# louiskirsch/speechT

Hardware: AMD Instinct MI355X
Metric: utterances/sec (training step, 10 s@16 kHz, batch 32) (higher is better)
Workload: dtype f32

## Files before the change

### include/speecht_hip.h

```cpp
#ifndef SPEECHT_HIP_H
#define SPEECHT_HIP_H

#include <stddef.h>
#include <stdint.h>

#ifdef __cplusplus
extern "C" {
#endif

#define ST_OK 0
#define ST_EINVAL (-1)
#define ST_ELAUNCH (-2)
#define ST_EWORKSPACE (-3)
#define ST_ECOMM (-4)

typedef struct st_tensor3 {
  float* base;
  int32_t batch;
  int32_t frames;
  int32_t channels;
  int32_t halo;
  int32_t t_pitch;
  int32_t c_pitch;
} st_tensor3;
// ... 10 lines not shown

int st_packed_dims(int width, int cin_pitch, int cout, int* k_valid, int* k_pad, int* n_pad);
int st_pack_filters_f32(const float* filters, int width, int cin, int cout, int cin_pitch,
                        float* packed, void* stream);
int st_unpack_filters_f32(const float* packed, int width, int cin, int cout, int cin_pitch,
                          float* filters, void* stream);
int st_filters_flip_transpose_f32(const float* packed, int width, int cin, int cout,
                                  int cin_pitch, int cout_pitch, float* packed_t, void* stream);

int st_conv1d_nwc_fwd_f32(const st_tensor3* x, const float* packed, const float* bias, int width,
                          int stride, int pad_left, int relu, const st_tensor3* y, void* stream);
size_t st_conv1d_fwd_ws(const st_tensor3* x, const st_tensor3* y, int width);
int st_conv1d_nwc_fwd_ws_f32(const st_tensor3* x, const float* packed, const float* bias, int width,
                             int stride, int pad_left, int relu, const st_tensor3* y, void* workspace,
                             size_t workspace_bytes, void* stream);

int st_conv1d_fft_plan(int width, int frames, int batch, int* n, int* valid, int* blocks, int* bins, int* rows_pad);
int st_gemm_nn_batched_f32(const float* a, int64_t lda, int64_t a_batch, const float* b, int64_t b_batch, float* c,
                           int64_t ldc, int64_t c_batch, int m, int k, int n, int batches, void* stream);
size_t st_gemm_nn_batched_ws_bytes(void);
size_t st_gemm_nn_batched_ctrl_bytes(void);
int st_streamk_lost_ptr(void** device_word);
int st_streamk_lost_count(unsigned* count);
int st_streamk_lost_fetch_async(unsigned* host_word, void* stream);
int st_gemm_nn_batched_ws_f32(const float* a, int64_t lda, int64_t a_batch, const float* b, int64_t b_batch, float* c,
                              int64_t ldc, int64_t c_batch, int m, int k, int n, int batches, void* workspace,
                              size_t workspace_bytes, void* stream);
int st_gemm_nn_batched_bt_ws_f32(const float* a, int64_t lda, int64_t a_batch, const float* bt, int64_t bt_batch, float* c,
                                 int64_t ldc, int64_t c_batch, int m, int k, int n, int batches, void* workspace,
                                 size_t workspace_bytes, void* stream);
// ... 51 lines not shown
                                      const float* tables, int planes, void* workspace, size_t workspace_bytes, void* stream);
int st_conv1d_nwc_bwd_filter_fft_planes(const st_tensor3* x, const st_tensor3* dz, const void* sf_planes, const void* zf_planes, int width,
                                        const float* tables, float* dpacked, int planes, void* workspace, size_t workspace_bytes,
                                        void* stream);

size_t st_conv1d_bwd_data_ws(const st_tensor3* dz, const st_tensor3* dx, int width);
int st_conv1d_nwc_bwd_data_f32(const st_tensor3* dz, const float* packed_t, int width,
                               int pad_left, const st_tensor3* act, const st_tensor3* dx,
                               void* workspace, size_t workspace_bytes, void* stream);
size_t st_conv1d_bwd_data_bias_ws(const st_tensor3* dz, const st_tensor3* dx, int width);
int st_conv1d_nwc_bwd_data_bias_f32(const st_tensor3* dz, const float* packed_t, int width, int pad_left,
                                    const st_tensor3* act, const st_tensor3* dx, float* dbias_dx,
                                    void* workspace, size_t workspace_bytes, void* stream);
int st_conv1d_1tap_bwd_data_bias_f32(const st_tensor3* dz, const float* packed, const st_tensor3* act, const st_tensor3* dx,
                                     float* dbias_dx, void* workspace, size_t workspace_bytes, void* stream);
size_t st_conv1d_bwd_filter_ws(const st_tensor3* x, const st_tensor3* dz, int width);
size_t st_bias_grad_ws(const st_tensor3* dz);
int st_bias_grad_f32(const st_tensor3* dz, float* dbias, void* workspace, size_t workspace_bytes, void* stream);
int st_conv1d_nwc_bwd_filter_f32(const st_tensor3* x, const st_tensor3* dz, int width, int stride,
                                 int pad_left, float* dpacked, float* dbias, void* workspace,
                                 size_t workspace_bytes, void* stream);

size_t st_ctc_ws(int batch, int frames, int max_label_len);
int st_ctc_loss_grad_f32(const st_tensor3* logits, const int32_t* label_ids,
                         const int32_t* label_offsets, const int32_t* seq_lens, int max_label_len,
                         float grad_scale, float* loss, const st_tensor3* grad, int32_t* status,
                         void* workspace, size_t workspace_bytes, void* stream);
int st_ctc_loss_grad_hilo_f32(const st_tensor3* logits, const int32_t* label_ids,
                              const int32_t* label_offsets, const int32_t* seq_lens, int max_label_len,
                              float grad_scale, float* loss, float* loss_lo, const st_tensor3* grad, int32_t* status,
// ... 144 lines not shown
```

### speecht_amd/_lib.py

```python
import ctypes
import os
from ctypes import POINTER, c_char_p, c_float, c_int, c_int32, c_int64, c_size_t, c_void_p

from .build import LIB_PATH


class Tensor3(ctypes.Structure):
  _fields_ = [('base', c_void_p), ('batch', c_int32), ('frames', c_int32), ('channels', c_int32),
              ('halo', c_int32), ('t_pitch', c_int32), ('c_pitch', c_int32)]


class SpeechtHipError(RuntimeError):
  pass


_T3P = POINTER(Tensor3)
_SIGNATURES = {
    'st_version': (c_int, []),
    'st_last_error': (c_char_p, []),
    'st_trace_begin': (c_int, []),
    'st_trace_begin_timed': (c_int, []),
    'st_trace_timed_filter': (c_int, [c_char_p]),
    'st_trace_end': (c_size_t, [c_char_p, c_size_t]),
    'st_set_tuning': (c_int, [c_char_p, c_int]),
    'st_host_crc32c': (ctypes.c_uint32, [c_void_p, c_size_t, ctypes.c_uint32]),
    'st_packed_dims': (c_int, [c_int, c_int, c_int, POINTER(c_int), POINTER(c_int), POINTER(c_int)]),
    'st_pack_filters_f32': (c_int, [c_void_p, c_int, c_int, c_int, c_int, c_void_p, c_void_p]),
    'st_unpack_filters_f32': (c_int, [c_void_p, c_int, c_int, c_int, c_int, c_void_p, c_void_p]),
    'st_filters_flip_transpose_f32': (c_int, [c_void_p, c_int, c_int, c_int, c_int, c_int, c_void_p, c_void_p]),
    'st_conv1d_nwc_fwd_f32': (c_int, [_T3P, c_void_p, c_void_p, c_int, c_int, c_int, c_int, _T3P, c_void_p]),
    'st_conv1d_fwd_ws': (c_size_t, [_T3P, _T3P, c_int]),
    'st_conv1d_nwc_fwd_ws_f32': (c_int, [_T3P, c_void_p, c_void_p, c_int, c_int, c_int, c_int, _T3P, c_void_p, c_size_t,
                                          c_void_p]),
    'st_conv1d_fft_plan': (c_int, [c_int, c_int, c_int, POINTER(c_int), POINTER(c_int), POINTER(c_int), POINTER(c_int),
                                   POINTER(c_int)]),
    'st_gemm_nn_batched_f32': (c_int, [c_void_p, c_int64, c_int64, c_void_p, c_int64, c_void_p, c_int64, c_int64, c_int, c_int,
                                       c_int, c_int, c_void_p]),
    'st_gemm_nn_batched_ws_bytes': (c_size_t, []),
    'st_gemm_nn_batched_ctrl_bytes': (c_size_t, []),
    'st_streamk_lost_ptr': (c_int, [POINTER(c_void_p)]),
    'st_streamk_lost_count': (c_int, [POINTER(ctypes.c_uint32)]),
    'st_streamk_lost_fetch_async': (c_int, [c_void_p, c_void_p]),
    'st_gemm_nn_batched_ws_f32': (c_int, [c_void_p, c_int64, c_int64, c_void_p, c_int64, c_void_p, c_int64, c_int64, c_int, c_int,
                                          c_int, c_int, c_void_p, c_size_t, c_void_p]),
    'st_gemm_nn_batched_bt_ws_f32': (c_int, [c_void_p, c_int64, c_int64, c_void_p, c_int64, c_void_p, c_int64, c_int64, c_int, c_int,
                                             c_int, c_int, c_void_p, c_size_t, c_void_p]),
    'st_gemm_tn_batched_f32': (c_int, [c_void_p, c_int64, c_int64, c_void_p, c_int64, c_int64, c_void_p, c_int64, c_int, c_int,
                                       c_int, c_int, c_void_p]),
# ... 28 lines not shown
                                                  c_void_p, c_size_t, c_void_p]),
    'st_conv1d_nwc_bwd_filter_fft_planes': (c_int, [_T3P, _T3P, c_void_p, c_void_p, c_int, c_void_p, c_void_p, c_int, c_void_p, c_size_t,
                                                    c_void_p]),
    'st_conv1d_fft_dz_spectra_f32': (c_int, [_T3P, c_int, c_void_p, c_void_p, c_void_p]),
    'st_conv1d_fft_bias_grad_f32': (c_int, [_T3P, c_int, c_void_p, c_void_p, c_void_p]),
    'st_conv1d_nwc_bwd_data_fft_f32': (c_int, [_T3P, c_void_p, c_void_p, c_int, c_int, _T3P, _T3P, c_void_p, c_void_p, c_size_t,
                                               c_void_p]),
    'st_conv1d_nwc_bwd_filter_fft_f32': (c_int, [_T3P, _T3P, c_void_p, c_void_p, c_int, c_void_p, c_void_p, c_void_p,
                                                 c_size_t, c_void_p]),
    'st_conv1d_bwd_data_ws': (c_size_t, [_T3P, _T3P, c_int]),
    'st_conv1d_nwc_bwd_data_f32': (c_int, [_T3P, c_void_p, c_int, c_int, _T3P, _T3P, c_void_p, c_size_t, c_void_p]),
    'st_conv1d_bwd_data_bias_ws': (c_size_t, [_T3P, _T3P, c_int]),
    'st_conv1d_nwc_bwd_data_bias_f32': (c_int, [_T3P, c_void_p, c_int, c_int, _T3P, _T3P, c_void_p, c_void_p, c_size_t,
                                                c_void_p]),
    'st_conv1d_1tap_bwd_data_bias_f32': (c_int, [_T3P, c_void_p, _T3P, _T3P, c_void_p, c_void_p, c_size_t, c_void_p]),
    'st_conv1d_bwd_filter_ws': (c_size_t, [_T3P, _T3P, c_int]),
    'st_conv1d_nwc_bwd_filter_f32': (c_int, [_T3P, _T3P, c_int, c_int, c_int, c_void_p, c_void_p, c_void_p,
                                             c_size_t, c_void_p]),
    'st_bias_grad_ws': (c_size_t, [_T3P]),
    'st_bias_grad_f32': (c_int, [_T3P, c_void_p, c_void_p, c_size_t, c_void_p]),
    'st_ctc_ws': (c_size_t, [c_int, c_int, c_int]),
    'st_ctc_loss_grad_f32': (c_int, [_T3P, c_void_p, c_void_p, c_void_p, c_int, c_float, c_void_p, _T3P,
                                     c_void_p, c_void_p, c_size_t, c_void_p]),
    'st_ctc_loss_grad_hilo_f32': (c_int, [_T3P, c_void_p, c_void_p, c_void_p, c_int, c_float, c_void_p, c_void_p, _T3P,
                                     c_void_p, c_void_p, c_size_t, c_void_p]),
    'st_ctc_greedy_decode': (c_int, [_T3P, c_void_p, c_int, c_void_p, c_int, c_void_p, c_void_p, c_void_p]),
    'st_ctc_align_ws': (c_size_t, [c_int, c_int, c_int]),
    'st_ctc_align_f32': (c_int, [_T3P, c_void_p, c_void_p, c_void_p, c_int, c_void_p, c_void_p, c_void_p, c_void_p,
                                 c_void_p, c_size_t, c_void_p]),
    'st_ctc_align_host': (c_int, [c_void_p, c_int, c_int, c_int, c_void_p, c_void_p, c_void_p, c_int, c_void_p, c_void_p,
# ... 159 lines not shown
```

### speecht_amd/csrc/conv_gemm.hip

```cpp
#include <algorithm>
#include <atomic>
#include <cmath>
#include <cstdlib>

#include <type_traits>

#include "st_common.h"
#include "streamk_map.h"

namespace {

typedef float f32x16 __attribute__((ext_vector_type(16)));
typedef float f32x4 __attribute__((ext_vector_type(4)));

constexpr int BK = 32;
constexpr int APITCH = BK + 4;
constexpr int NTHREADS = 256;

struct RowMap {
  int frames;
  int row_stride;
  long batch_stride;
  long row0;
  __device__ __forceinline__ long off(int m) const {
// ... 8 lines not shown
  const float* Bm; int Np;
  float* C;        RowMap cmap;
  const float* mask; RowMap mmap;
  const float* bias;
  int M, Kvalid, Kp, n_store, relu;
  int taps, cp;
  int tiles_m, tiles_n, chunk;
  int gm, tm_per, tn_per;
  int splits, steps_per_split;
  float* slab;
  float* colsum;
  int colsum_rows;
  int batches;
  long a_batch, b_batch, c_batch;
  long bt_ld; int bt_rows;
};


__device__ __forceinline__ void dma16_sv(unsigned lds_byte_addr, const void* sbase, unsigned voff_bytes) {
  unsigned keep;
  asm volatile("s_mov_b32 %0, m0\n\ts_mov_b32 m0, %1\n\ts_nop 0\n\tglobal_load_lds_dwordx4 %2, %3\n\ts_mov_b32 m0, %0"
               : "=&s"(keep) : "s"(lds_byte_addr), "v"(voff_bytes), "s"(sbase) : "memory");
}
__device__ __forceinline__ void dma_wait_all() { asm volatile("s_waitcnt vmcnt(0)" ::: "memory"); }
__device__ __forceinline__ unsigned lds_addr(const float* p) {
  return (unsigned)(size_t)(__attribute__((address_space(3))) const float*)p;
}

template <int N> struct FVec;
template <> struct FVec<1> { typedef float type; };
// ... 89 lines not shown
  for (; kt + 2 < nk; kt += 2) {
    stage(integral_constant<int, 0>{}, true_type{});
    stage(integral_constant<int, 1>{}, true_type{});
  }
  if (kt + 2 == nk) {
    stage(integral_constant<int, 0>{}, true_type{});
    stage(integral_constant<int, 1>{}, false_type{});
  } else if (kt + 1 == nk) {
    stage(integral_constant<int, 0>{}, false_type{});
  }
}

template <int BM, int BN, int WMW, int WNW, int EPI, bool FAST = false, bool BT = false>
__global__ __launch_bounds__(NTHREADS) void gemm_nn_kernel(NNParams p) {
  static_assert(!BT || FAST, "the transposed-operand variant exists for whole k-tiles only");
  typedef NNStage<BM, BN, WMW, WNW, BT> S;
  constexpr int WTM = S::WTM, WTN = S::WTN, MT = S::MT, NT = S::NT;
  constexpr int A_DMA = S::A_DMA, B_DMA = S::B_DMA, N_DMA = S::N_DMA, A_SZ = S::A_SZ, B_SZ = S::B_SZ;
  constexpr int B_LPR = BN / 4;
  static_assert(WMW * WNW == 4 && MT >= 1 && (NT == 1 || NT == 2 || NT == 4) && A_DMA >= 1 && B_DMA >= 1, "tile config");
  typedef typename FVec<NT>::type bvec;

  __shared__ __attribute__((aligned(16))) float smem[2 * A_SZ + 2 * B_SZ + 6 * BM];
  float* const As = smem;
  float* const Bs = smem + 2 * A_SZ;
  long* const a_off = reinterpret_cast<long*>(smem + 2 * A_SZ + 2 * B_SZ);
  long* const c_off = a_off + BM;
  long* const m_off = c_off + BM;

  const int bid = blockIdx.x;
// ... 130 lines not shown
        for (int r = 0; r < 16; ++r) {
          const int m = m0 + wm * WTM + i * 32 + (r & 3) + 8 * (r >> 2) + 4 * h;
          if (m < p.M) {
#pragma unroll
            for (int n = 0; n < NT; ++n) slab[(long)m * p.Np + colb + n * 32] = acc[i][n][r];
          }
        }
      return;
    }
    float csum[NT], bv[NT];
    bool ok[NT];
#pragma unroll
    for (int n = 0; n < NT; ++n) {
      ok[n] = colb + n * 32 < p.n_store;
      csum[n] = 0.f;
      bv[n] = (EPI == 0 && p.bias && ok[n]) ? p.bias[colb + n * 32] : 0.f;
    }
#pragma unroll
    for (int i = 0; i < MT; ++i) {
      float mk[16][NT];
      if (EPI == 1 && p.mask) {
#pragma unroll
        for (int r = 0; r < 16; ++r) {
          const int row = wm * WTM + i * 32 + (r & 3) + 8 * (r >> 2) + 4 * h;
#pragma unroll
          for (int n = 0; n < NT; ++n) mk[r][n] = p.mask[m_off[row] + (ok[n] ? colb + n * 32 : 0)];
        }
      }
#pragma unroll
      for (int r = 0; r < 16; ++r) {
        const int row = wm * WTM + i * 32 + (r & 3) + 8 * (r >> 2) + 4 * h;
        const long co = c_off[row];
#pragma unroll
        for (int n = 0; n < NT; ++n) {
          float v = acc[i][n][r];
          if (EPI == 0) {
            v += bv[n];
            if (p.relu) v = fmaxf(v, 0.f);
          } else if (p.mask) {
            v = mk[r][n] > 0.f ? v : 0.f;
          }
          if (co >= 0 && ok[n]) {
            if (EPI == 1) csum[n] += v;
            Cbase[co + colb + n * 32] = v;
          }
        }
      }
    }
    if (EPI == 1 && p.colsum) {
#pragma unroll
      for (int n = 0; n < NT; ++n) {
// ... 14 lines not shown
        if (m < p.M) {
          bvec out;
#pragma unroll
          for (int n = 0; n < NT; ++n) vset<NT>(out, n, acc[i][n][r]);
          *reinterpret_cast<bvec*>(slab + (long)m * p.Np + col0) = out;
        }
      }
    return;
  }
  const bool col_ok = col0 < p.n_store;
  float csum[NT];
#pragma unroll
  for (int n = 0; n < NT; ++n) csum[n] = 0.f;
  bvec bv;
#pragma unroll
  for (int n = 0; n < NT; ++n) vset<NT>(bv, n, (EPI == 0 && p.bias && col_ok) ? p.bias[col0 + n] : 0.f);
#pragma unroll
  for (int i = 0; i < MT; ++i) {
    bvec mk[16];
    if (EPI == 1 && p.mask) {
      const int colc = col_ok ? col0 : 0;
#pragma unroll
      for (int r = 0; r < 16; ++r) {
        const int row = wm * WTM + i * 32 + (r & 3) + 8 * (r >> 2) + 4 * h;
        mk[r] = *reinterpret_cast<const bvec*>(p.mask + m_off[row] + colc);
      }
    }
#pragma unroll
    for (int r = 0; r < 16; ++r) {
      const int row = wm * WTM + i * 32 + (r & 3) + 8 * (r >> 2) + 4 * h;
      const long co = c_off[row];
      if (co >= 0 && col_ok) {
        bvec out;
#pragma unroll
        for (int n = 0; n < NT; ++n) {
          float v = acc[i][n][r];
          if (EPI == 0) {
            v += vget<NT>(bv, n);
            if (p.relu) v = fmaxf(v, 0.f);
          } else if (p.mask) {
            v = vget<NT>(mk[r], n) > 0.f ? v : 0.f;
          }
          if (EPI == 1) csum[n] += v;
          vset<NT>(out, n, v);
        }
        *reinterpret_cast<bvec*>(Cbase + co + col0) = out;
      }
    }
  }
  if (EPI == 1 && p.colsum) {
    bvec out;
#pragma unroll
    for (int n = 0; n < NT; ++n) vset<NT>(out, n, csum[n] + __shfl_xor(csum[n], 32, 64));
    if (h == 0) *reinterpret_cast<bvec*>(p.colsum + (long)(tile_m * WMW + wm) * p.Np + col0) = out;
  }
}

__device__ unsigned g_sk_lost = 0;

struct BinsParams {
  const float* A; const float* B; float* C;
  long lda, ldb, ldc, a_batch, b_batch, c_batch;
// ... 785 lines not shown
    const float* src = p.slab + (long)m * p.Np + c4;
    f32x4 v = *reinterpret_cast<const f32x4*>(src);
    for (int sidx = 1; sidx < p.splits; ++sidx) v += *reinterpret_cast<const f32x4*>(src + (long)sidx * p.M * p.Np);
    if (epi == 0) {
      if (p.bias) v += *reinterpret_cast<const f32x4*>(p.bias + c4);
      if (p.relu) { v[0] = fmaxf(v[0], 0.f); v[1] = fmaxf(v[1], 0.f); v[2] = fmaxf(v[2], 0.f); v[3] = fmaxf(v[3], 0.f); }
    } else if (p.mask) {
      f32x4 mk = *reinterpret_cast<const f32x4*>(p.mask + p.mmap.off(m) + c4);
#pragma unroll
      for (int e = 0; e < 4; ++e) v[e] = mk[e] > 0.f ? v[e] : 0.f;
    }
    *reinterpret_cast<f32x4*>(p.C + p.cmap.off(m) + c4) = v;
  }
}

int nn_splits(int M, int Np, int Kp) {
  if (Np % 128) return 1;
  const long tiles128 = (long)st::ceil_div(M, 128) * (Np / 128);
  const int nk = Kp / BK;
  int splits = tiles128 < 64 && nk >= 256 ? (int)std::min<long>(8, 256 / tiles128)
                                          : (tiles128 > 128 && tiles128 <= 320 && nk >= 512 ? 2 : 1);
  while (splits > 1 && nk / splits < 64) --splits;
  return splits;
}

int fwd_splits(int M, int Np, int nk) {
  if (Np == 32) {
    if (M < 1024 || nk < 32) return 1;
    const int tiles_m = st::ceil_div(M, 128);
    return std::max(1, std::min(std::min(8, nk / 4), (512 + tiles_m / 2) / tiles_m));
// ... 25 lines not shown
    p.chunk = p.tm_per * p.tn_per;
  }
  p.colsum_rows = p.tiles_m * WMW;
  if (p.batches > 0) p.chunk = st::ceil_div(p.batches, 8) * p.tiles_m * p.tiles_n;
  dim3 grid(p.chunk * 8, p.splits > 1 ? p.splits : 1), block(NTHREADS);
  const double gflop = 2e-9 * p.tiles_m * BM * (double)p.Np * p.Kp * std::max(1, p.batches);
  if (p.batches > 0)
    st::trace("gemm_nn<%d,%d,%d,%d,%s> batched bins=%d M=%d Np=%d Kp=%d gflop=%.3f", BM, BN, WMW, WNW, FAST ? (BT ? "fast-bt" : "fast") : "clamped",
              p.batches, p.M, p.Np, p.Kp, gflop);
  else
    st::trace("gemm_nn<%d,%d,%d,%d,%s> epi=%d splits=%d M=%d Np=%d Kp=%d taps=%d xcd=%dx%d gflop=%.3f", BM, BN, WMW, WNW,
              FAST ? (BT ? "fast-bt" : "fast") : "clamped", epi, p.splits > 1 ? p.splits : 1, p.M, p.Np, p.Kp, p.taps, p.gm, 8 / p.gm, gflop);
  {
    st::LaunchTimer timer(s);
    if (epi == 0) st::launch_timed(timer, gemm_nn_kernel<BM, BN, WMW, WNW, 0, FAST, BT>, grid, block, s, p);
    else st::launch_timed(timer, gemm_nn_kernel<BM, BN, WMW, WNW, 1, FAST, BT>, grid, block, s, p);
  }
  if (p.splits > 1) {
    const long quads = (long)p.M * (p.n_store / 4);
    hipLaunchKernelGGL(splitk_epilogue_kernel, dim3((unsigned)std::min<long>((quads + 255) / 256, 4096)), dim3(256), 0, s,
                       p, epi);
  }
}

int run_nn(NNParams& p, int epi, hipStream_t s) {
  if (p.bt_ld > 0) {
    if (!(p.Np % 128 == 0 && p.taps == 1 && p.cp % 32 == 0 && p.Kvalid % 32 == 0 && p.Kvalid == p.Kp && p.bt_ld % 4 == 0 && p.bt_rows > 0)) {
      st::set_error("gemm_nn: the transposed-operand form needs n_pad %% 128 == 0, one tap and a reduction length that is a multiple of 32");
      return ST_EINVAL;
    }
    const long tiles128 = (long)st::ceil_div(p.M, 128) * (p.Np / 128) * std::max(1, p.batches);
    if ((p.batches > 0 && (tiles128 < 512 || p.M <= 64)) || (p.batches <= 0 && tiles128 < 192 && p.splits <= 1)) launch_nn<64, 128, 2, 2, true, true>(p, epi, s);
    else launch_nn<128, 128, 2, 2, true, true>(p, epi, s);
// ... 176 lines not shown
  TN3Params p{};
  p.A = A; p.lda = lda; p.a_batch = a_batch;
  p.Z = Z; p.ldz = ldz; p.z_batch = z_batch;
  for (int i = 0; i < 3; ++i) { p.a_off[i] = a_off[i]; p.z_off[i] = z_off[i]; }
  p.out = out; p.o_batch = o_batch; p.o_part = o_part;
  p.M = M; p.K = K; p.N = N; p.tiles_k = K / 128; p.tiles_n = N / 128; p.batches = batches;
  st::trace("gemm_tn_g3<128> batched bins=%d M=%d Kp=%d Np=%d gflop=%.3f", batches, M, K, N, 2e-9 * 3 * M * (double)K * N * batches);
  st::LaunchTimer timer(s);
  st::launch_timed(timer, gemm_tn_g3_kernel, dim3(st::ceil_div(batches, 8) * p.tiles_k * p.tiles_n * 8), dim3(TN_THREADS), s, p);
  return st::check_launch("gemm_tn_g3_batched");
}

static int bwd_data_impl(const st_tensor3* dz, const float* packed_t, bool forward_filters, int width, int pad_left,
                         const st_tensor3* act, const st_tensor3* dx, float* dbias_dx, void* workspace,
                         size_t workspace_bytes, void* stream);

extern "C" {

int st_streamk_lost_ptr(void** device_word) {
  ST_REQUIRE(device_word, "st_streamk_lost_ptr: null argument");
  void* p = nullptr;
  if (hipGetSymbolAddress(&p, HIP_SYMBOL(g_sk_lost)) != hipSuccess || !p) {
    st::set_error("st_streamk_lost_ptr: hipGetSymbolAddress failed");
    return ST_ELAUNCH;
  }
  *device_word = p;
  return ST_OK;
}

int st_streamk_lost_fetch_async(unsigned* host_word, void* stream) {
// ... 94 lines not shown
  const int np = st::npad_of(y->channels);
  const int M = y->batch * y->frames;
  const int nk = width > 1 ? st::ceil_div(x->c_pitch, BK) * width : st::ceil_div(x->c_pitch, BK);
  const int splits = fwd_splits(M, np, nk);
  return splits > 1 ? (size_t)splits * M * np * sizeof(float) : 0;
}

int st_conv1d_nwc_fwd_f32(const st_tensor3* x, const float* packed, const float* bias, int width,
                          int stride, int pad_left, int relu, const st_tensor3* y, void* stream) {
  return st_conv1d_nwc_fwd_ws_f32(x, packed, bias, width, stride, pad_left, relu, y, nullptr, 0, stream);
}

int st_conv1d_nwc_fwd_ws_f32(const st_tensor3* x, const float* packed, const float* bias, int width,
                             int stride, int pad_left, int relu, const st_tensor3* y, void* workspace,
                             size_t workspace_bytes, void* stream) {
  ST_REQUIRE(st::tensor_ok(x) && st::tensor_ok(y) && packed, "conv fwd: bad tensor descriptor");
  ST_REQUIRE(width > 0 && stride > 0 && pad_left >= 0 && x->batch == y->batch, "conv fwd: bad shape");
  ST_REQUIRE(y->frames == st::ceil_div(x->frames, stride), "conv fwd: y.frames != ceil(x.frames/stride)");
  ST_REQUIRE(x->halo >= pad_left, "conv fwd: x.halo %d < pad_left %d", x->halo, pad_left);
  ST_REQUIRE((y->frames - 1) * stride + width - pad_left <= x->t_pitch - x->halo,
             "conv fwd: trailing halo of x too small");
  NNParams p{};
  p.A = x->base;
  p.amap = make_map(*x, x->halo - pad_left, stride, y->frames);
  p.Bm = packed;
  p.Np = st::npad_of(y->channels);
  p.C = y->base;
  p.cmap = make_map(*y, y->halo, 1, y->frames);
  p.bias = bias;
  p.M = y->batch * y->frames;
  p.Kvalid = width * x->c_pitch;
  p.Kp = (int)st::round_up(p.Kvalid, BK);
  p.n_store = std::min(y->c_pitch, p.Np);
  p.relu = relu;
  p.taps = width;
  p.cp = x->c_pitch;
  const int nk = p.taps > 1 ? st::ceil_div(p.cp, BK) * p.taps : p.Kp / BK;
  const int splits = fwd_splits(p.M, p.Np, nk);
  if (splits > 1 && workspace && workspace_bytes >= (size_t)splits * p.M * p.Np * sizeof(float)) {
    p.steps_per_split = st::ceil_div(nk, splits);
    p.splits = st::ceil_div(nk, p.steps_per_split);
    p.slab = reinterpret_cast<float*>(workspace);
  }
  return run_nn(p, 0, st::as_stream(stream));
}

size_t st_conv1d_bwd_data_ws(const st_tensor3* dz, const st_tensor3* dx, int width) {
  if (!dz || !dx) return 0;
  const int np = st::npad_of(dx->channels), kp = (int)st::round_up((size_t)width * dz->c_pitch, BK);
  const int M = dx->batch * dx->frames;
  const int splits = nn_splits(M, np, kp);
  return splits > 1 ? (size_t)splits * M * np * sizeof(float) : 0;
}

int st_conv1d_nwc_bwd_data_f32(const st_tensor3* dz, const float* packed_t, int width, int pad_left,
                               const st_tensor3* act, const st_tensor3* dx, void* workspace,
                               size_t workspace_bytes, void* stream) {
  return st_conv1d_nwc_bwd_data_bias_f32(dz, packed_t, width, pad_left, act, dx, nullptr, workspace, workspace_bytes, stream);
}

// ... 4 lines not shown
  return st::round_up(st_conv1d_bwd_data_ws(dz, dx, width), 256) + rows * np * sizeof(float) + 256;
}

int st_conv1d_nwc_bwd_data_bias_f32(const st_tensor3* dz, const float* packed_t, int width, int pad_left,
                                    const st_tensor3* act, const st_tensor3* dx, float* dbias_dx, void* workspace,
                                    size_t workspace_bytes, void* stream) {
  return bwd_data_impl(dz, packed_t, false, width, pad_left, act, dx, dbias_dx, workspace, workspace_bytes, stream);
}

int st_conv1d_1tap_bwd_data_bias_f32(const st_tensor3* dz, const float* packed, const st_tensor3* act, const st_tensor3* dx,
                                     float* dbias_dx, void* workspace, size_t workspace_bytes, void* stream) {
  ST_REQUIRE(st::tensor_ok(dz) && st::tensor_ok(dx) && dz->c_pitch % 32 == 0 && st::npad_of(dx->channels) % 128 == 0 &&
                 st::npad_of(dz->channels) >= dz->c_pitch,
             "conv 1-tap bwd_data: needs a channel pitch of dz that is a multiple of 32 and an input width that packs to 128s");
  return bwd_data_impl(dz, packed, true, 1, 0, act, dx, dbias_dx, workspace, workspace_bytes, stream);
}

}

static int bwd_data_impl(const st_tensor3* dz, const float* packed_t, bool forward_filters, int width, int pad_left,
                         const st_tensor3* act, const st_tensor3* dx, float* dbias_dx, void* workspace,
                         size_t workspace_bytes, void* stream) {
  ST_REQUIRE(st::tensor_ok(dz) && st::tensor_ok(dx) && packed_t, "conv bwd_data: bad tensor descriptor");
  ST_REQUIRE(dz->batch == dx->batch && dz->frames == dx->frames, "conv bwd_data: stride-1 layers only");
  const int lead = width - 1 - pad_left;
  ST_REQUIRE(lead >= 0 && dz->halo >= lead, "conv bwd_data: dz.halo %d < %d", dz->halo, lead);
  ST_REQUIRE(dz->frames + pad_left <= dz->t_pitch - dz->halo, "conv bwd_data: trailing halo of dz too small");
  if (act) ST_REQUIRE(st::tensor_ok(act) && act->batch == dx->batch && act->frames == dx->frames &&
                      act->c_pitch >= std::min(dx->c_pitch, st::npad_of(dx->channels)),
                      "conv bwd_data: mask tensor mismatch");
// ... 162 lines not shown
```

### speecht_amd/modes/fp32.py

```python
import ctypes
import os
from types import SimpleNamespace

import torch

from .. import _lib
from .._lib import call
from .base import ModeBase
from .spectral import SpectralLayers


class Fp32Mode(SpectralLayers, ModeBase):
  _one_tap_in_place = True
  _flip_every_layer = False
  masks_padding = True

  def __init__(self, engine):
    super().__init__(engine)
    self._packed_t_fresh, self._packed_t_layers, self._bwd_ready = False, frozenset(), {}
    self._gfwd_fresh, self._gfwd_ready, self._fft_table_key, self._fft_prev = False, {}, {}, None

  def weights_changed(self):
    self._packed_t_fresh = False
    self._gfwd_fresh = False
# ... 3 lines not shown

  def alloc(self, sh):
    lib, e, part = _lib.load(), self.e, SimpleNamespace()
    ws = self._workspace_bytes(lib, sh)
    part.wgrad_ws, _ = e._storage.view('wgrad_ws', ws // 4 + 64)
    top = len(e.layers) - 1
    part.side_wgrad_top = (self._top_gradient_beside and e.side_filter_gradient and os.environ.get('ST_WGRAD_SIDE_TOP', '1') != '0' and
                           top > 0 and e.layers[top].cout <= 64 and e.layers[top].width == 1)
    part.wgrad_ws_top = None
    if part.side_wgrad_top:
      ws_top = lib.st_conv1d_bwd_filter_ws(sh.X[top].ref, sh.dZ[top].ref, e.layers[top].width)
      part.wgrad_ws_top, _ = e._storage.view('wgrad_ws_top', ws_top // 4 + 64)
    part.fft_layers = {i for i in range(len(e.layers)) if self._use_fft(i, sh.batch, sh.geo)}
    self._alloc_planes(sh, part)
    self._alloc_fft(sh, part)
    return part

  _top_gradient_beside = True

  def reenter(self, sh):
    self._fft_transition(sh.mode.fft, sh.mode.table_keys)

  def _workspace_bytes(self, lib, sh):
    layers, X, dZ = self.e.layers, sh.X, sh.dZ
    ws = max(lib.st_conv1d_bwd_filter_ws(X[i].ref, dZ[i].ref, l.width) for i, l in enumerate(layers))
    ws = max([ws] + [lib.st_conv1d_bwd_data_bias_ws(dZ[i].ref, dZ[i - 1].ref, l.width) for i, l in enumerate(layers) if i > 0])
    return max([ws] + [lib.st_conv1d_fwd_ws(X[i].ref, X[i + 1].ref, l.width) for i, l in enumerate(layers)])

  def _x6_fwd(self, part, i):
    return False
  _x6_bwd = _x6_wgrad = _x6_fwd
# ... 71 lines not shown
        self._x6_forward_layer(i, pb)
      elif i in fft:
        f = fft[i]
        if not self._gfwd_fresh:
          e._join_side_stream()
          self._refresh_fft_filters()
        self._wait_gfwd(i)
        nxt = None if mask_padding else fft.get(i + 1)
        if nxt is not None and nxt['shift'] is not None:
          nxt = None
        written = ctypes.c_int(0)
        call('st_conv1d_nwc_fwd_fft_chain_f32', f['xref'], ptr(f['gfwd']), ptr(pb), f['width'], f['pl'], int(l.relu), X[i + 1].ref,
             ptr(f['tables']), ptr(f['sf']), int(sf_ready), ptr(nxt['tables']) if nxt else None, ptr(nxt['sf']) if nxt else None,
             nxt['width'] if nxt else 0, nxt['pl'] if nxt else 0, ctypes.byref(written), ptr(f['ws']), f['ws'].numel() * 4, s)
        sf_ready = written.value == 1
      else:
        call('st_conv1d_nwc_fwd_ws_f32', X[i].ref, ptr(pf), ptr(pb), l.width, l.stride, geo[i][2], int(l.relu), X[i + 1].ref,
             ptr(ws), ws_bytes, s)
      if mask_padding and i < top:
        call('st_mask_rows', X[i + 1].ref, valid(i), 4, s)

  def backward(self, on_layer_done, wanted):
    e, ptr, sh, s, layers = self.e, self.e._ptr, self.e.shape, self.e.stream_ptr, self.e.layers
    X, dZ, geo, part = sh.X, sh.dZ, sh.geo, sh.mode
    fft = part.fft if e.fft_conv else {}
    wgrad_ws, wgrad_ws_bytes = part.wgrad_ws, part.wgrad_ws.numel() * 4
    if not self._packed_t_ok():
      self._refresh_backward_operands()
    if fft and not self._gfwd_fresh:
      e._join_side_stream()
# ... 1 lines not shown
    self._wait_gfwd()
    self._backward_prologue()
    wait_all_below = len(layers) - 3
    side_wgrad, deferred = False, None
    top_pending = None
    hook = on_layer_done
    if hook is not None:
      def on_layer_done(j):
        nonlocal top_pending
        if top_pending is not None and top_pending != j:
          e._join_side_stream(second_only=True)
          hook(top_pending)
          top_pending = None
        if top_pending != j:
          hook(j)
    bias_from_above = False
    zf_ready = False
    for i in reversed(range(len(layers))):
      l = layers[i]
      gf, gb = e._slice(e.grads, i)
      need_bias, bias_from_above = not bias_from_above, False
      if self._x6_wgrad(part, i):
        self._x6_filter_gradient(i, gf, gb, need_bias)
      elif i in fft:
        f = fft[i]
        if not zf_ready:
          call('st_conv1d_fft_dz_spectra_f32', dZ[i].ref, f['width'], ptr(f['tables']), ptr(f['zf']), s)
        zf_ready = False
        polyphase = f['shift'] is not None

# ... 27 lines not shown
          side_wgrad = False
        on_layer_done(i)
      if i > 0 and self._x6_bwd(part, i):
        self._x6_back_prop(i)
      elif i > 0 and i in fft:
        f = fft[i]
        act = X[i].ref if layers[i - 1].relu else None
        below = part.fft.get(i - 1)
        written = ctypes.c_int(0)
        call('st_conv1d_nwc_bwd_data_fft_chain_f32', dZ[i].ref, ptr(f['zf']), ptr(f['gfwd']), l.width, geo[i][2], act,
             dZ[i - 1].ref, ptr(f['tables']), ptr(below['tables']) if below else None, ptr(below['zf']) if below else None,
             below['width'] if below else 0, ctypes.byref(written), ptr(f['ws']), f['ws'].numel() * 4, s)
        zf_ready = written.value == 1
      elif i > 0:
        act = X[i].ref if layers[i - 1].relu else None
        if self._transposed_in_place(i):
          call('st_conv1d_1tap_bwd_data_bias_f32', dZ[i].ref, ptr(e._slice(e.params, i)[0]), act, dZ[i - 1].ref,
               ptr(e._slice(e.grads, i - 1)[1]), ptr(wgrad_ws), wgrad_ws_bytes, s)
        else:
          self._wait_bwd_operands(i if i > wait_all_below else None)
          call('st_conv1d_nwc_bwd_data_bias_f32', dZ[i].ref, ptr(e.packed_t[i]), l.width, geo[i][2], act, dZ[i - 1].ref,
               ptr(e._slice(e.grads, i - 1)[1]), ptr(wgrad_ws), wgrad_ws_bytes, s)
        bias_from_above = True
      if deferred == i and on_layer_done is not None and wanted(i):
        e._join_side_stream()
        side_wgrad = False
        on_layer_done(i)
      if deferred == i:
        deferred = None
    if side_wgrad or top_pending is not None:
      e._join_side_stream()
# ... 3 lines not shown
```

Baseline: 4855.

## Pack top-layer ReLU mask into bits in forward epilogue for 1-tap backward

The forward GEMM epilogue for the layer feeding the top 1-tap conv gains a variant that writes a 1-bit-per-element ReLU mask alongside the activation, using wave ballots (plus a split-K epilogue variant). A dedicated 1-tap backward-data kernel then reads this compact mask instead of the full f32 activation to gate the gradient, and also produces the bias column sums. This aims to cut backward memory traffic for the widest activation read. It adds mask storage, a new kernel, and layout constraints (channel pitch of 32, output widths that pack to 128s).

```diff
diff --git a/include/speecht_hip.h b/include/speecht_hip.h
--- a/include/speecht_hip.h
+++ b/include/speecht_hip.h
@@ -48,6 +48,11 @@
 int st_conv1d_nwc_fwd_ws_f32(const st_tensor3* x, const float* packed, const float* bias, int width,
                              int stride, int pad_left, int relu, const st_tensor3* y, void* workspace,
                              size_t workspace_bytes, void* stream);
+size_t st_relu_bits_bytes(const st_tensor3* y);
+int st_relu_bits_pack_host(const float* act, long rows, int channels, long row_stride, int c_pitch, void* relu_bits);
+int st_conv1d_nwc_fwd_ws_bits_f32(const st_tensor3* x, const float* packed, const float* bias, int width,
+                                  int stride, int pad_left, int relu, const st_tensor3* y, void* relu_bits, void* workspace,
+                                  size_t workspace_bytes, void* stream);
 
 int st_conv1d_fft_plan(int width, int frames, int batch, int* n, int* valid, int* blocks, int* bins, int* rows_pad);
 int st_gemm_nn_batched_f32(const float* a, int64_t lda, int64_t a_batch, const float* b, int64_t b_batch, float* c,
@@ -129,6 +134,9 @@
                                     void* workspace, size_t workspace_bytes, void* stream);
 int st_conv1d_1tap_bwd_data_bias_f32(const st_tensor3* dz, const float* packed, const st_tensor3* act, const st_tensor3* dx,
                                      float* dbias_dx, void* workspace, size_t workspace_bytes, void* stream);
+size_t st_conv1d_1tap_bwd_data_bits_ws(const st_tensor3* dx);
+int st_conv1d_1tap_bwd_data_bits_f32(const st_tensor3* dz, const float* packed, const void* relu_bits, const st_tensor3* dx,
+                                     float* dbias_dx, void* workspace, size_t workspace_bytes, void* stream);
 size_t st_conv1d_bwd_filter_ws(const st_tensor3* x, const st_tensor3* dz, int width);
 size_t st_bias_grad_ws(const st_tensor3* dz);
 int st_bias_grad_f32(const st_tensor3* dz, float* dbias, void* workspace, size_t workspace_bytes, void* stream);
diff --git a/speecht_amd/_lib.py b/speecht_amd/_lib.py
--- a/speecht_amd/_lib.py
+++ b/speecht_amd/_lib.py
@@ -32,6 +32,10 @@
     'st_conv1d_fwd_ws': (c_size_t, [_T3P, _T3P, c_int]),
     'st_conv1d_nwc_fwd_ws_f32': (c_int, [_T3P, c_void_p, c_void_p, c_int, c_int, c_int, c_int, _T3P, c_void_p, c_size_t,
                                           c_void_p]),
+    'st_relu_bits_bytes': (c_size_t, [_T3P]),
+    'st_relu_bits_pack_host': (c_int, [c_void_p, c_int64, c_int, c_int64, c_int, c_void_p]),
+    'st_conv1d_nwc_fwd_ws_bits_f32': (c_int, [_T3P, c_void_p, c_void_p, c_int, c_int, c_int, c_int, _T3P, c_void_p, c_void_p, c_size_t,
+                                               c_void_p]),
     'st_conv1d_fft_plan': (c_int, [c_int, c_int, c_int, POINTER(c_int), POINTER(c_int), POINTER(c_int), POINTER(c_int),
                                    POINTER(c_int)]),
     'st_gemm_nn_batched_f32': (c_int, [c_void_p, c_int64, c_int64, c_void_p, c_int64, c_void_p, c_int64, c_int64, c_int, c_int,
@@ -90,6 +94,8 @@
     'st_conv1d_nwc_bwd_data_bias_f32': (c_int, [_T3P, c_void_p, c_int, c_int, _T3P, _T3P, c_void_p, c_void_p, c_size_t,
                                                 c_void_p]),
     'st_conv1d_1tap_bwd_data_bias_f32': (c_int, [_T3P, c_void_p, _T3P, _T3P, c_void_p, c_void_p, c_size_t, c_void_p]),
+    'st_conv1d_1tap_bwd_data_bits_ws': (c_size_t, [_T3P]),
+    'st_conv1d_1tap_bwd_data_bits_f32': (c_int, [_T3P, c_void_p, c_void_p, _T3P, c_void_p, c_void_p, c_size_t, c_void_p]),
     'st_conv1d_bwd_filter_ws': (c_size_t, [_T3P, _T3P, c_int]),
     'st_conv1d_nwc_bwd_filter_f32': (c_int, [_T3P, _T3P, c_int, c_int, c_int, c_void_p, c_void_p, c_void_p,
                                              c_size_t, c_void_p]),
diff --git a/speecht_amd/csrc/conv_gemm.hip b/speecht_amd/csrc/conv_gemm.hip
--- a/speecht_amd/csrc/conv_gemm.hip
+++ b/speecht_amd/csrc/conv_gemm.hip
@@ -6,6 +6,7 @@
 #include <type_traits>
 
 #include "st_common.h"
+#include "relu_bits.h"
 #include "streamk_map.h"
 
 namespace {
@@ -46,6 +47,7 @@
   int batches;
   long a_batch, b_batch, c_batch;
   long bt_ld; int bt_rows;
+  unsigned* bits; int bit_groups;
 };
 
 
@@ -165,6 +167,7 @@
 template <int BM, int BN, int WMW, int WNW, int EPI, bool FAST = false, bool BT = false>
 __global__ __launch_bounds__(NTHREADS) void gemm_nn_kernel(NNParams p) {
   static_assert(!BT || FAST, "the transposed-operand variant exists for whole k-tiles only");
+  constexpr bool FWD = EPI != 1, BITS = EPI == 2;
   typedef NNStage<BM, BN, WMW, WNW, BT> S;
   constexpr int WTM = S::WTM, WTN = S::WTN, MT = S::MT, NT = S::NT;
   constexpr int A_DMA = S::A_DMA, B_DMA = S::B_DMA, N_DMA = S::N_DMA, A_SZ = S::A_SZ, B_SZ = S::B_SZ;
@@ -325,7 +328,7 @@
     for (int n = 0; n < NT; ++n) {
       ok[n] = colb + n * 32 < p.n_store;
       csum[n] = 0.f;
-      bv[n] = (EPI == 0 && p.bias && ok[n]) ? p.bias[colb + n * 32] : 0.f;
+      bv[n] = (FWD && p.bias && ok[n]) ? p.bias[colb + n * 32] : 0.f;
     }
 #pragma unroll
     for (int i = 0; i < MT; ++i) {
@@ -345,7 +348,7 @@
 #pragma unroll
         for (int n = 0; n < NT; ++n) {
           float v = acc[i][n][r];
-          if (EPI == 0) {
+          if (FWD) {
             v += bv[n];
             if (p.relu) v = fmaxf(v, 0.f);
           } else if (p.mask) {
@@ -390,7 +393,7 @@
   for (int n = 0; n < NT; ++n) csum[n] = 0.f;
   bvec bv;
 #pragma unroll
-  for (int n = 0; n < NT; ++n) vset<NT>(bv, n, (EPI == 0 && p.bias && col_ok) ? p.bias[col0 + n] : 0.f);
+  for (int n = 0; n < NT; ++n) vset<NT>(bv, n, (FWD && p.bias && col_ok) ? p.bias[col0 + n] : 0.f);
 #pragma unroll
   for (int i = 0; i < MT; ++i) {
     bvec mk[16];
@@ -402,26 +405,42 @@
         mk[r] = *reinterpret_cast<const bvec*>(p.mask + m_off[row] + colc);
       }
     }
+    uint2 bw = {0u, 0u};
 #pragma unroll
     for (int r = 0; r < 16; ++r) {
       const int row = wm * WTM + i * 32 + (r & 3) + 8 * (r >> 2) + 4 * h;
       const long co = c_off[row];
+      bool pos[NT] = {};
       if (co >= 0 && col_ok) {
         bvec out;
 #pragma unroll
         for (int n = 0; n < NT; ++n) {
           float v = acc[i][n][r];
-          if (EPI == 0) {
+          if (FWD) {
             v += vget<NT>(bv, n);
             if (p.relu) v = fmaxf(v, 0.f);
           } else if (p.mask) {
             v = vget<NT>(mk[r], n) > 0.f ? v : 0.f;
           }
           if (EPI == 1) csum[n] += v;
+          if (BITS) pos[n] = v > 0.f;
           vset<NT>(out, n, v);
         }
         *reinterpret_cast<bvec*>(Cbase + co + col0) = out;
       }
+      if constexpr (BITS) {
+        static_assert(!BITS || (NT == 2 && WTN == st::RB_GROUP), "the bit mask needs 64-column wave tiles");
+        const unsigned long long b0 = __ballot(pos[0]), b1 = __ballot(pos[NT - 1]);
+        const bool mine = r == (l31 & 3) + 4 * (l31 >> 3), upper = (l31 & 4) != 0;
+        const unsigned x = upper ? (unsigned)(b0 >> 32) : (unsigned)b0, y = upper ? (unsigned)(b1 >> 32) : (unsigned)b1;
+        bw.x = mine ? x : bw.x;
+        bw.y = mine ? y : bw.y;
+      }
+    }
+    if constexpr (BITS) {
+      const int rl = wm * WTM + i * 32 + l31, grp = (n0 + wn * WTN) / st::RB_GROUP;
+      if (h == 0 && c_off[rl] >= 0 && grp < p.bit_groups)
+        *reinterpret_cast<uint2*>(p.bits + st::rb_group_word(m0 + rl, grp, p.M)) = bw;
     }
   }
   if (EPI == 1 && p.colsum) {
@@ -1237,6 +1256,142 @@
   }
 }
 
+__device__ __forceinline__ unsigned rb_spread16(unsigned x) {
+  x = (x | (x << 8)) & 0x00ff00ffu;
+  x = (x | (x << 4)) & 0x0f0f0f0fu;
+  x = (x | (x << 2)) & 0x33333333u;
+  return (x | (x << 1)) & 0x55555555u;
+}
+__global__ __launch_bounds__(256) void splitk_epilogue_bits_kernel(NNParams p) {
+  const int quads = p.bit_groups * 16;
+  const long total = (long)p.M * quads;
+  const int lane = threadIdx.x & 63;
+  for (long idx = (long)blockIdx.x * 256 + threadIdx.x; idx < total; idx += (long)gridDim.x * 256) {
+    const int m = (int)(idx / quads), q = (int)(idx % quads), c4 = q * 4;
+    const bool ok = c4 < p.n_store;
+    f32x4 v = {0.f, 0.f, 0.f, 0.f};
+    if (ok) {
+      const float* src = p.slab + (long)m * p.Np + c4;
+      v = *reinterpret_cast<const f32x4*>(src);
+      for (int sidx = 1; sidx < p.splits; ++sidx) v += *reinterpret_cast<const f32x4*>(src + (long)sidx * p.M * p.Np);
+      if (p.bias) v += *reinterpret_cast<const f32x4*>(p.bias + c4);
+      if (p.relu) { v[0] = fmaxf(v[0], 0.f); v[1] = fmaxf(v[1], 0.f); v[2] = fmaxf(v[2], 0.f); v[3] = fmaxf(v[3], 0.f); }
+      *reinterpret_cast<f32x4*>(p.C + p.cmap.off(m) + c4) = v;
+    }
+    unsigned e[4];
+#pragma unroll
+    for (int k = 0; k < 4; ++k) e[k] = (unsigned)(__ballot(ok && v[k] > 0.f) >> (16 * (lane >> 4))) & 0xffffu;
+    if ((lane & 15) == 0) {
+      uint2 w;
+      w.x = rb_spread16(e[0]) | (rb_spread16(e[2]) << 1);
+      w.y = rb_spread16(e[1]) | (rb_spread16(e[3]) << 1);
+      *reinterpret_cast<uint2*>(p.bits + st::rb_group_word(m, q / 16, p.M)) = w;
+    }
+  }
+}
+
+constexpr unsigned RB1_NO_ROW = 0xffffffffu;
+constexpr int RB1_PANEL_GROUPS = 4;
+struct RB1Params {
+  const float* dz; RowMap zmap;
+  const float* Bt; int bt_rows;
+  float* dx; RowMap xmap;
+  const unsigned* bits; int bit_groups;
+  float* colsum;
+  int rows32;
+  int M, n_store, Np, panels, panel_groups;
+};
+
+__global__ __launch_bounds__(NTHREADS, 4) void relu_bwd_1tap_kernel(RB1Params p) {
+  __shared__ __attribute__((aligned(16))) float Bs[RB1_PANEL_GROUPS * 64 * BK + 128 + RB1_PANEL_GROUPS * 128 * 2];
+  unsigned* const c_off = reinterpret_cast<unsigned*>(Bs + RB1_PANEL_GROUPS * 64 * BK);
+  uint2* const mask_s = reinterpret_cast<uint2*>(c_off + 128);
+  const int tile_m = blockIdx.x / p.panels, panel = blockIdx.x - tile_m * p.panels;
+  const int tid = threadIdx.x;
+  const int lane = tid & 63;
+  const int wave = __builtin_amdgcn_readfirstlane(tid >> 6);
+  const int l31 = lane & 31, h = lane >> 5;
+  const int wm = wave >> 1, wn = wave & 1;
+  const int g0 = panel * p.panel_groups;
+  const int ng = min(p.panel_groups, p.Np / 64 - g0);
+
+  for (int idx = tid; idx < ng * 64 * 8; idx += NTHREADS) {
+    const int cl = idx >> 3, k4 = (idx & 7) * 4;
+    const int c = cl & 63;
+    const int row = (cl & ~63) + (c & 1) * 32 + (c >> 1);
+    const f32x4 w = *reinterpret_cast<const f32x4*>(p.Bt + (long)min(g0 * 64 + cl, p.bt_rows - 1) * 32 + k4);
+    *reinterpret_cast<f32x4*>(Bs + row * BK + ((((idx & 7) ^ ((row >> 1) & 7))) * 4)) = w;
+  }
+
+  if (tid < 128) {
+    const int m = tile_m * 128 + tid;
+    c_off[tid] = m < p.M ? (unsigned)p.xmap.off(m) : RB1_NO_ROW;
+  }
+  for (int idx = tid; idx < ng * 128; idx += NTHREADS) {
+    const int gl = idx >> 7, m = tile_m * 128 + (idx & 127), g = g0 + gl;
+    uint2 w = make_uint2(~0u, ~0u);
+    if (p.bits) w = (m < p.M && g < p.bit_groups) ? *reinterpret_cast<const uint2*>(p.bits + st::rb_group_word(m, g, p.M)) : make_uint2(0u, 0u);
+    mask_s[idx] = w;
+  }
+  const int mw = tile_m * 128 + wm * 64;
+  f32x4 af[2][4];
+#pragma unroll
+  for (int i = 0; i < 2; ++i) {
+    const float* src = p.dz + p.zmap.off(min(mw + i * 32 + l31, p.M - 1)) + 4 * h;
+#pragma unroll
+    for (int q = 0; q < 4; ++q) af[i][q] = *reinterpret_cast<const f32x4*>(src + 8 * q);
+  }
+  __syncthreads();
+
+  float* __restrict__ dx = p.dx;
+  for (int gl = wn; gl < ng; gl += 2) {
+    const int g = g0 + gl;
+    const int col0 = g * 64 + 2 * l31;
+    const bool ok = col0 < p.n_store;
+    float csum[2] = {0.f, 0.f};
+#pragma unroll 1
+    for (int i = 0; i < 2; ++i) {
+      f32x16 acc0 = {}, acc1 = {};
+#pragma unroll
+      for (int q = 0; q < 4; ++q) {
+        const f32x4 b0 = *reinterpret_cast<const f32x4*>(Bs + swz_frag(gl * 64 + l31, q, h));
+        const f32x4 b1 = *reinterpret_cast<const f32x4*>(Bs + swz_frag(gl * 64 + 32 + l31, q, h));
+        const f32x4 a = i ? af[1][q] : af[0][q];
+#pragma unroll
+        for (int j = 0; j < 4; ++j) {
+          acc0 = __builtin_amdgcn_mfma_f32_32x32x2f32(a[j], b0[j], acc0, 0, 0, 0);
+          acc1 = __builtin_amdgcn_mfma_f32_32x32x2f32(a[j], b1[j], acc1, 0, 0, 0);
+        }
+      }
+#pragma unroll
+      for (int r = 0; r < 16; ++r) {
+        const int row = wm * 64 + i * 32 + (r & 3) + 8 * (r >> 2) + 4 * h;
+        const uint2 mk = mask_s[gl * 128 + row];
+        const unsigned co = c_off[row];
+        float v0 = acc0[r], v1 = acc1[r];
+        v0 = (mk.x >> l31) & 1u ? v0 : 0.f;
+        v1 = (mk.y >> l31) & 1u ? v1 : 0.f;
+        if (co != RB1_NO_ROW && ok) {
+          csum[0] += v0;
+          csum[1] += v1;
+          FVec<2>::type out;
+          out[0] = v0;
+          out[1] = v1;
+          *reinterpret_cast<FVec<2>::type*>(dx + (co + (unsigned)col0)) = out;
+        }
+      }
+      if (p.colsum && (p.rows32 || i == 1)) {
+        FVec<2>::type out;
+        out[0] = csum[0] + __shfl_xor(csum[0], 32, 64);
+        out[1] = csum[1] + __shfl_xor(csum[1], 32, 64);
+        const int block = p.rows32 ? (tile_m * 2 + wm) * 2 + i : tile_m * 2 + wm;
+        if (h == 0) *reinterpret_cast<FVec<2>::type*>(p.colsum + (long)block * p.Np + col0) = out;
+        csum[0] = csum[1] = 0.f;
+      }
+    }
+  }
+}
+
 int nn_splits(int M, int Np, int Kp) {
   if (Np % 128) return 1;
   const long tiles128 = (long)st::ceil_div(M, 128) * (Np / 128);
@@ -1292,9 +1447,13 @@
   {
     st::LaunchTimer timer(s);
     if (epi == 0) st::launch_timed(timer, gemm_nn_kernel<BM, BN, WMW, WNW, 0, FAST, BT>, grid, block, s, p);
-    else st::launch_timed(timer, gemm_nn_kernel<BM, BN, WMW, WNW, 1, FAST, BT>, grid, block, s, p);
-  }
-  if (p.splits > 1) {
+    else if (epi == 1) st::launch_timed(timer, gemm_nn_kernel<BM, BN, WMW, WNW, 1, FAST, BT>, grid, block, s, p);
+    else if constexpr (BN == 128 && WNW == 2 && !BT) st::launch_timed(timer, gemm_nn_kernel<BM, BN, WMW, WNW, 2, FAST, BT>, grid, block, s, p);
+  }
+  if (p.splits > 1 && epi == 2) {
+    const long quads = (long)p.M * p.bit_groups * 16;
+    hipLaunchKernelGGL(splitk_epilogue_bits_kernel, dim3((unsigned)std::min<long>((quads + 255) / 256, 4096)), dim3(256), 0, s, p);
+  } else if (p.splits > 1) {
     const long quads = (long)p.M * (p.n_store / 4);
     hipLaunchKernelGGL(splitk_epilogue_kernel, dim3((unsigned)std::min<long>((quads + 255) / 256, 4096)), dim3(256), 0, s,
                        p, epi);
@@ -1501,6 +1660,8 @@
 static int bwd_data_impl(const st_tensor3* dz, const float* packed_t, bool forward_filters, int width, int pad_left,
                          const st_tensor3* act, const st_tensor3* dx, float* dbias_dx, void* workspace,
                          size_t workspace_bytes, void* stream);
+static int fwd_impl(const st_tensor3* x, const float* packed, const float* bias, int width, int stride, int pad_left, int relu,
+                    const st_tensor3* y, unsigned* relu_bits, void* workspace, size_t workspace_bytes, void* stream);
 
 extern "C" {
 
@@ -1625,6 +1786,35 @@
 int st_conv1d_nwc_fwd_ws_f32(const st_tensor3* x, const float* packed, const float* bias, int width,
                              int stride, int pad_left, int relu, const st_tensor3* y, void* workspace,
                              size_t workspace_bytes, void* stream) {
+  return fwd_impl(x, packed, bias, width, stride, pad_left, relu, y, nullptr, workspace, workspace_bytes, stream);
+}
+
+size_t st_relu_bits_bytes(const st_tensor3* y) {
+  return y ? st::rb_bytes((long)y->batch * y->frames, y->c_pitch) : 0;
+}
+
+int st_relu_bits_pack_host(const float* act, long rows, int channels, long row_stride, int c_pitch, void* relu_bits) {
+  ST_REQUIRE(act && relu_bits && rows >= 0 && channels > 0 && channels <= c_pitch && row_stride >= channels, "st_relu_bits_pack_host: bad args");
+  unsigned* w = reinterpret_cast<unsigned*>(relu_bits);
+  for (size_t i = 0; i < st::rb_bytes(rows, c_pitch) / sizeof(unsigned); ++i) w[i] = 0u;
+  for (long m = 0; m < rows; ++m)
+    for (int c = 0; c < channels; ++c)
+      if (act[m * row_stride + c] > 0.f) w[st::rb_word(m, c, rows)] |= 1u << st::rb_bit(c);
+  return ST_OK;
+}
+
+int st_conv1d_nwc_fwd_ws_bits_f32(const st_tensor3* x, const float* packed, const float* bias, int width,
+                                  int stride, int pad_left, int relu, const st_tensor3* y, void* relu_bits, void* workspace,
+                                  size_t workspace_bytes, void* stream) {
+  ST_REQUIRE(relu_bits && ((uintptr_t)relu_bits & 7) == 0 && y && st::npad_of(y->channels) % 128 == 0,
+             "conv fwd (bit mask): needs a mask buffer and an output width that packs to 128s");
+  return fwd_impl(x, packed, bias, width, stride, pad_left, relu, y, reinterpret_cast<unsigned*>(relu_bits), workspace, workspace_bytes, stream);
+}
+
+}
+
+static int fwd_impl(const st_tensor3* x, const float* packed, const float* bias, int width, int stride, int pad_left, int relu,
+                    const st_tensor3* y, unsigned* relu_bits, void* workspace, size_t workspace_bytes, void* stream) {
   ST_REQUIRE(st::tensor_ok(x) && st::tensor_ok(y) && packed, "conv fwd: bad tensor descriptor");
   ST_REQUIRE(width > 0 && stride > 0 && pad_left >= 0 && x->batch == y->batch, "conv fwd: bad shape");
   ST_REQUIRE(y->frames == st::ceil_div(x->frames, stride), "conv fwd: y.frames != ceil(x.frames/stride)");
@@ -1653,8 +1843,14 @@
     p.splits = st::ceil_div(nk, p.steps_per_split);
     p.slab = reinterpret_cast<float*>(workspace);
   }
-  return run_nn(p, 0, st::as_stream(stream));
-}
+  if (relu_bits) {
+    p.bits = relu_bits;
+    p.bit_groups = st::rb_groups(y->c_pitch);
+  }
+  return run_nn(p, relu_bits ? 2 : 0, st::as_stream(stream));
+}
+
+extern "C" {
 
 size_t st_conv1d_bwd_data_ws(const st_tensor3* dz, const st_tensor3* dx, int width) {
   if (!dz || !dx) return 0;
@@ -1689,6 +1885,54 @@
                  st::npad_of(dz->channels) >= dz->c_pitch,
              "conv 1-tap bwd_data: needs a channel pitch of dz that is a multiple of 32 and an input width that packs to 128s");
   return bwd_data_impl(dz, packed, true, 1, 0, act, dx, dbias_dx, workspace, workspace_bytes, stream);
+}
+
+size_t st_conv1d_1tap_bwd_data_bits_ws(const st_tensor3* dx) {
+  if (!dx) return 0;
+  return (size_t)st::ceil_div(dx->batch * dx->frames, 128) * 4 * st::npad_of(dx->channels) * sizeof(float) + 256;
+}
+
+int st_conv1d_1tap_bwd_data_bits_f32(const st_tensor3* dz, const float* packed, const void* relu_bits, const st_tensor3* dx,
+                                     float* dbias_dx, void* workspace, size_t workspace_bytes, void* stream) {
+  ST_REQUIRE(st::tensor_ok(dz) && st::tensor_ok(dx) && packed && dz->c_pitch == 32 && st::npad_of(dz->channels) == 32 &&
+                 st::npad_of(dx->channels) % 128 == 0 && dz->batch == dx->batch && dz->frames == dx->frames,
+             "conv 1-tap bwd_data (bit mask): needs a dz channel pitch of 32 and an input width that packs to 128s");
+  ST_REQUIRE(((uintptr_t)relu_bits & 7) == 0, "conv 1-tap bwd_data (bit mask): the mask must be 8-byte aligned");
+  ST_REQUIRE((size_t)dx->batch * dx->t_pitch * dx->c_pitch < ((size_t)1 << 30), "conv 1-tap bwd_data (bit mask): dx of 4 GiB or more");
+  ST_REQUIRE(!dbias_dx || (workspace && workspace_bytes >= st_conv1d_1tap_bwd_data_bits_ws(dx)),
+             "conv 1-tap bwd_data (bit mask): workspace too small for the bias gradient");
+  hipStream_t s = st::as_stream(stream);
+  RB1Params p{};
+  p.dz = dz->base;
+  p.zmap = make_map(*dz, dz->halo, 1, dx->frames);
+  p.Bt = packed;
+  p.bt_rows = dx->c_pitch;
+  p.dx = dx->base;
+  p.xmap = make_map(*dx, dx->halo, 1, dx->frames);
+  p.bits = reinterpret_cast<const unsigned*>(relu_bits);
+  p.bit_groups = st::rb_groups(dx->c_pitch);
+  p.M = dx->batch * dx->frames;
+  p.Np = st::npad_of(dx->channels);
+  p.n_store = std::min(dx->c_pitch, p.Np);
+  p.colsum = dbias_dx ? reinterpret_cast<float*>(workspace) : nullptr;
+  const int tiles_m = st::ceil_div(p.M, 128), groups = p.Np / 64;
+  p.rows32 = (long)tiles_m * (p.Np / 128) < 192;
+  const int colsum_rows = p.rows32 ? st::ceil_div(p.M, 64) * 2 : tiles_m * 2;
+  p.panel_groups = RB1_PANEL_GROUPS;
+  while (p.panel_groups > 2 && tiles_m * st::ceil_div(groups, p.panel_groups) <= 512) p.panel_groups -= 2;
+  p.panels = st::ceil_div(groups, p.panel_groups);
+  const double mb = 1e-6 * ((double)p.M * p.n_store * 4 + (p.bits ? (double)st::rb_bytes(p.M, dx->c_pitch) : 0.0) + (double)p.M * 32 * 4);
+  st::trace("relu_bwd_1tap rows=%d cols=%d panels=%d gflop=%.3f mb=%.2f", p.M, p.n_store, p.panels, 2e-9 * tiles_m * 128 * (double)p.Np * 32, mb);
+  {
+    st::LaunchTimer timer(s);
+    st::launch_timed(timer, relu_bwd_1tap_kernel, dim3(tiles_m * p.panels), dim3(NTHREADS), s, p);
+  }
+  if (int e = st::check_launch("relu_bwd_1tap")) return e;
+  if (dbias_dx) {
+    hipLaunchKernelGGL(colsum_final_kernel, dim3(st::ceil_div(p.Np, 32)), dim3(256), 0, s, p.colsum, colsum_rows, p.Np, dbias_dx);
+    return st::check_launch("relu_bwd_1tap bias gradient");
+  }
+  return ST_OK;
 }
 
 }
diff --git a/speecht_amd/csrc/relu_bits.h b/speecht_amd/csrc/relu_bits.h
--- /dev/null
+++ b/speecht_amd/csrc/relu_bits.h
@@ -0,0 +1,22 @@
+#pragma once
+
+#include <stddef.h>
+#include <stdint.h>
+
+#ifdef __HIPCC__
+#define ST_RB_HD __host__ __device__ __forceinline__
+#else
+#define ST_RB_HD inline
+#endif
+
+namespace st {
+
+constexpr int RB_GROUP = 64;
+
+ST_RB_HD int rb_groups(int c_pitch) { return (c_pitch + RB_GROUP - 1) / RB_GROUP; }
+ST_RB_HD long rb_group_word(long row, int group, long rows) { return (group * rows + row) * 2; }
+ST_RB_HD long rb_word(long row, int channel, long rows) { return rb_group_word(row, channel / RB_GROUP, rows) + (channel & 1); }
+ST_RB_HD int rb_bit(int channel) { return (channel % RB_GROUP) >> 1; }
+ST_RB_HD size_t rb_bytes(long rows, int c_pitch) { return (size_t)rows * rb_groups(c_pitch) * 2 * sizeof(uint32_t); }
+
+}
diff --git a/speecht_amd/modes/fp32.py b/speecht_amd/modes/fp32.py
--- a/speecht_amd/modes/fp32.py
+++ b/speecht_amd/modes/fp32.py
@@ -41,7 +41,21 @@
     part.fft_layers = {i for i in range(len(e.layers)) if self._use_fft(i, sh.batch, sh.geo)}
     self._alloc_planes(sh, part)
     self._alloc_fft(sh, part)
+    part.relu_bits, part.relu_bits_ws, part.relu_bits_current = None, None, False
+    if self._relu_bits_top_ok(part, top):
+      part.relu_bits, _ = e._storage.view('relu_bits_top', lib.st_relu_bits_bytes(sh.X[top].ref) // 4 + 2)
+      part.relu_bits_ws, _ = e._storage.view('relu_bits_top_ws', lib.st_conv1d_1tap_bwd_data_bits_ws(sh.dZ[top - 1].ref) // 4 + 64)
     return part
+
+  _relu_bits_top = True
+
+  def _relu_bits_top_ok(self, part, top):
+    layers = self.e.layers
+    if not (self._relu_bits_top and top > 0 and self._transposed_in_place(top)):
+      return False
+    l, below = layers[top], layers[top - 1]
+    return (l.cout_pitch == 32 and l.n_pad == 32 and bool(below.relu) and top not in part.fft_layers and top - 1 not in part.fft_layers and
+            not self._x6_fwd(part, top - 1) and not self._x6_bwd(part, top))
 
   _top_gradient_beside = True
 
@@ -143,6 +157,10 @@
              ptr(f['tables']), ptr(f['sf']), int(sf_ready), ptr(nxt['tables']) if nxt else None, ptr(nxt['sf']) if nxt else None,
              nxt['width'] if nxt else 0, nxt['pl'] if nxt else 0, ctypes.byref(written), ptr(f['ws']), f['ws'].numel() * 4, s)
         sf_ready = written.value == 1
+      elif part.relu_bits is not None and i + 2 == len(e.layers):
+        part.relu_bits_current = not mask_padding
+        call('st_conv1d_nwc_fwd_ws_bits_f32', X[i].ref, ptr(pf), ptr(pb), l.width, l.stride, geo[i][2], int(l.relu), X[i + 1].ref,
+             ptr(part.relu_bits), ptr(ws), ws_bytes, s)
       else:
         call('st_conv1d_nwc_fwd_ws_f32', X[i].ref, ptr(pf), ptr(pb), l.width, l.stride, geo[i][2], int(l.relu), X[i + 1].ref,
              ptr(ws), ws_bytes, s)
@@ -174,6 +192,7 @@
           top_pending = None
         if top_pending != j:
           hook(j)
+    bits_top = part.relu_bits is not None and part.relu_bits_current
     bias_from_above = False
     zf_ready = False
     for i in reversed(range(len(layers))):
@@ -231,7 +250,10 @@
         zf_ready = written.value == 1
       elif i > 0:
         act = X[i].ref if layers[i - 1].relu else None
-        if self._transposed_in_place(i):
+        if bits_top and i + 1 == len(layers):
+          call('st_conv1d_1tap_bwd_data_bits_f32', dZ[i].ref, ptr(e._slice(e.params, i)[0]), ptr(part.relu_bits), dZ[i - 1].ref,
+               ptr(e._slice(e.grads, i - 1)[1]), ptr(part.relu_bits_ws), part.relu_bits_ws.numel() * 4, s)
+        elif self._transposed_in_place(i):
           call('st_conv1d_1tap_bwd_data_bias_f32', dZ[i].ref, ptr(e._slice(e.params, i)[0]), act, dZ[i - 1].ref,
                ptr(e._slice(e.grads, i - 1)[1]), ptr(wgrad_ws), wgrad_ws_bytes, s)
         else:
```

New measurement: 4494. 0.926x the previous value.
